# fightingnoble/rram-caffe-simulation

Measured on AMD Instinct MI355X. Metric: Monte Carlo fault-map inferences/sec, AlexNet b256, higher is better.
Workload: dtype f32 (bf16x6 products)

## Files before the change

rram-caffe-simulation_amd/csrc/x6.hip:

```cpp
#include <stdio.h>
#include <stdlib.h>
#include <string.h>

#include <algorithm>
#include <atomic>
#include <string>
#include <type_traits>

#include "gemm_common.hpp"
#include "split3.hpp"

namespace rram {
namespace {

#ifndef RRAM_X6_DROP
#define RRAM_X6_DROP 0
#endif
namespace x6 {
__device__ __forceinline__ floatx16 mfma6(const Parts& a, const Parts& b, floatx16 c) {
  if (RRAM_X6_DROP != 1) c = __builtin_amdgcn_mfma_f32_32x32x16_bf16(a.l, b.h, c, 0, 0, 0);
  if (RRAM_X6_DROP != 2) c = __builtin_amdgcn_mfma_f32_32x32x16_bf16(a.h, b.l, c, 0, 0, 0);
  if (RRAM_X6_DROP != 3) c = __builtin_amdgcn_mfma_f32_32x32x16_bf16(a.m, b.m, c, 0, 0, 0);
  if (RRAM_X6_DROP != 4) c = __builtin_amdgcn_mfma_f32_32x32x16_bf16(a.m, b.h, c, 0, 0, 0);
  if (RRAM_X6_DROP != 5) c = __builtin_amdgcn_mfma_f32_32x32x16_bf16(a.h, b.m, c, 0, 0, 0);
// ... 1059 lines not shown
  static_assert(NS * STB + 1024 <= 160 * 1024, "LDS");
  static_assert((NS - 2) * PPW <= 63, "vmcnt");
  __shared__ __attribute__((aligned(16))) char smem[NS * STB + 1024];
  const uint32_t lds0 = static_cast<uint32_t>(reinterpret_cast<uintptr_t>((__attribute__((address_space(3))) char*)smem));

  const int lane = threadIdx.x & 63;
  const int wave = __builtin_amdgcn_readfirstlane(threadIdx.x >> 6);
  const int lr = lane & 31, lh = lane >> 5;
  const int wr = wave % WR, wc = wave / WR;
  const int tid = xcd_tile_id(blockIdx.x, gridDim.x);
  const int tm = __builtin_amdgcn_readfirstlane(tid % P.tiles_m);
  const int tn = __builtin_amdgcn_readfirstlane(tid / P.tiles_m);
  const int m0 = tm * BMc, n0 = tn * BNc;
  const int HW = static_cast<int>(P.cv.howo.d), C = P.cv.C, KT = C >> 4;
  const int4v xrs = make_rsrc(x, xrange);
  const int4v wrs = make_rsrc(reinterpret_cast<const float*>(wpack), wrange);
  uint32_t aoff[PA], alds[PA];
#pragma unroll
  for (int i = 0; i < PA; ++i) {
    const int a = wave + 4 * i;
    const bool ok = a < NA;
    aoff[i] = ok ? static_cast<uint32_t>(((tm * RBL + a / 3) * KT) * 3072 + (a % 3) * 1024 + lane * 16) : 0x80000000u;
    alds[i] = ok ? static_cast<uint32_t>((a / 3 * 3 + a % 3) * 1024) : 0xFFFFFFFFu;
  }
  uint32_t boff[PB], blds[PB];
#pragma unroll
  for (int i = 0; i < PB; ++i) {
    const int q = wave + 4 * i;
    uint32_t off = 0x80000000u;
    if (q < NBP) {
      const int e = q * (PIECE_B / 4) + lane * 4;
      const int c = e / BNc, n = n0 + (e - c * BNc);
      if (n < P.N) {
        const uint32_t img = fdiv(static_cast<uint32_t>(n), P.cv.howo);
        const uint32_t sp = static_cast<uint32_t>(n) - img * static_cast<uint32_t>(HW);
        off = ((img * static_cast<uint32_t>(C) + static_cast<uint32_t>(c)) * static_cast<uint32_t>(HW) + sp) * 4u;
      }
    }
    boff[i] = off;
    blds[i] = q < NBP ? static_cast<uint32_t>(A_BYTES + q * PIECE_B) : 0xFFFFFFFFu;
  }
  const uint32_t kstep = static_cast<uint32_t>(HW) * 64u;
  auto issue = [&](int kt) {
    const bool ok = kt < KT;
    const uint32_t st = lds0 + static_cast<uint32_t>((kt % NS) * STB);
#pragma unroll
    for (int i = 0; i < PA; ++i) {
      const bool real = ok && alds[i] != 0xFFFFFFFFu;
      dma_b128(wrs, real ? aoff[i] + static_cast<uint32_t>(kt) * 3072u : 0x80000000u,
               real ? st + alds[i] : lds0 + static_cast<uint32_t>(NS * STB));
    }
#pragma unroll
    for (int i = 0; i < PB; ++i) {
      const bool real = ok && blds[i] != 0xFFFFFFFFu;
      const uint32_t vo = real && boff[i] != 0x80000000u ? boff[i] + static_cast<uint32_t>(kt) * kstep : 0x80000000u;
      const uint32_t dst = real ? st + blds[i] : lds0 + static_cast<uint32_t>(NS * STB);
      dma_b128(xrs, vo, dst);
    }
  };
  floatx16 acc[MI][NB];
#pragma unroll
  for (int i = 0; i < MI; ++i)
#pragma unroll
    for (int j = 0; j < NB; ++j)
#pragma unroll
      for (int r = 0; r < 16; ++r) acc[i][j][r] = 0.0f;

#pragma unroll
  for (int t = 0; t < NS - 1; ++t) issue(t);
  wait_vm<(NS - 2) * PPW>();
  __builtin_amdgcn_s_barrier();
  const int colw = 32 * NB * wc + lr;
  for (int kt = 0; kt < KT; ++kt) {
    issue(kt + NS - 1);
    const char* st = smem + (kt % NS) * STB;
    x6::Parts fa[MI];
#pragma unroll
    for (int i = 0; i < MI; ++i) {
      const char* f = st + (MI * wr + i) * 3072 + lane * 16;
      fa[i].h = *reinterpret_cast<const x6::bf16x8*>(f);
      fa[i].m = *reinterpret_cast<const x6::bf16x8*>(f + 1024);
      fa[i].l = *reinterpret_cast<const x6::bf16x8*>(f + 2048);
    }
    const float* bs = reinterpret_cast<const float*>(st + A_BYTES) + 8 * lh * BNc + colw;
#pragma unroll
    for (int j = 0; j < NB; ++j) {
      float v[8];
#pragma unroll
      for (int e = 0; e < 8; ++e) v[e] = bs[e * BNc + 32 * j];
      x6::Parts bp;
      x6::split8_safe(v, bp);
#pragma unroll
      for (int i = 0; i < MI; ++i) acc[i][j] = x6::mfma6(fa[i], bp, acc[i][j]);
    }
    wait_vm<(NS - 2) * PPW>();
    asm volatile("s_waitcnt lgkmcnt(0)" ::: "memory");
    __builtin_amdgcn_s_barrier();
    __builtin_amdgcn_sched_barrier(0);
  }
  Epi ep = P.e;
  conv_epilogue_nchw<MI, NB>(acc, P, ep, m0 + 32 * MI * wr, n0 + 32 * NB * wc, lr, lh);
  if (yoct != nullptr) octet_epilogue<MI, NB>(acc, P, ep, m0 + 32 * MI * wr, n0 + 32 * NB * wc, lr, lh, yoct, cout8);
}

__global__ void __launch_bounds__(256) k_conv_cb_pack_x6(const float* __restrict__ w, char* __restrict__ out, int M,
                                                         int Cg, int T, int rblocks, int units) {
  const int KT = Cg >> 4;
  for (int u = blockIdx.x * blockDim.x + threadIdx.x; u < units; u += gridDim.x * blockDim.x) {
    const int lane = u & 63;
    int r = u >> 6;
    const int s = r % T;
    r /= T;
    const int kt = r % KT;
    r /= KT;
    const int rb = r % rblocks;
    const int g = r / rblocks;
    const int m = rb * 32 + (lane & 31), c0 = kt * 16 + (lane >> 5) * 8;
    float v[8];
#pragma unroll
    for (int e = 0; e < 8; ++e)
      v[e] = m < M ? w[((int64_t)g * M + m) * Cg * T + (int64_t)(c0 + e) * T + s] : 0.0f;
    x6::Parts t;
    x6::split8_safe(v, t);
    char* f = out + (int64_t)(u >> 6) * 3072 + lane * 16;
    *reinterpret_cast<x6::bf16x8*>(f) = t.h;
    *reinterpret_cast<x6::bf16x8*>(f + 1024) = t.m;
    *reinterpret_cast<x6::bf16x8*>(f + 2048) = t.l;
  }
}


namespace c1x6 {
constexpr int BM = 96, BN = 256;
constexpr int KR = 11, KQ = 3, C = 3, NQ = C * KR * KQ, G = (NQ + 3) / 4;
constexpr int ROWS = 32;
constexpr int ROWE = 248;
constexpr int TERMB = ROWS * ROWE * 2;
constexpr int SLOTB = 3 * TERMB;
constexpr int QP = ROWE / 8;
constexpr int CHUNKS = ROWS * QP;
constexpr int CPT = (CHUNKS + 255) / 256;
static_assert(3 * SLOTB + BM * 4 <= 160 * 1024, "LDS");
constexpr int first_group(int c) { return (c * KR * KQ) / 4; }
constexpr int last_group(int c) { return (c * KR * KQ + KR * KQ - 1) / 4; }
constexpr int quad_off(int q) {
  return (q / (KR * KQ)) * SLOTB + (((q / KQ) % KR) * ROWE + 4 * (q % KQ)) * 2;
}
constexpr int half_delta(int q) { return q + 1 < NQ ? quad_off(q + 1) - quad_off(q) : 0; }
constexpr uint32_t hi_mask(int q) { return q >= NQ ? 0u : (q % KQ == KQ - 1 ? 0x0000FFFFu : 0xFFFFFFFFu); }
constexpr uint32_t lo_mask(int q) { return q >= NQ ? 0u : 0xFFFFFFFFu; }
}

template <int W>
__global__ void __launch_bounds__(256) __attribute__((amdgpu_waves_per_eu(1, 1)))
k_conv1_ring_x6(Params P, const uint16_t* __restrict__ wpack, int tiles_per_img, int tiles) {
  using namespace c1x6;
  constexpr int OW = (W - 11) / 4 + 1, MI = 3;
  static_assert(4 * (OW - 1) + 4 * KQ <= ROWE, "slot rows too short");
  __shared__ __attribute__((aligned(16))) char smem[3 * SLOTB];
  __shared__ float bias_lds[BM];
  if (threadIdx.x < BM)
    bias_lds[threadIdx.x] = (P.e.bias != nullptr && (int)threadIdx.x < P.M) ? P.e.bias[threadIdx.x] : 0.0f;
  const int lane = threadIdx.x & 63;
  const int wave = __builtin_amdgcn_readfirstlane(threadIdx.x >> 6);
  const int lr = lane & 31, lh = lane >> 5;
  const int HWo = P.cv.howo.d, H = P.cv.H;
  const int nwg = gridDim.x;
  const float* const xin = P.b.p;
  const int in_bytes = static_cast<int>(P.cv.in_bytes);

  float sv[2][8];
  struct TileRef {
    int img, f;
  };
  auto tile_ref = [&](int t) __attribute__((always_inline)) {
    TileRef r;
    const int img = t / tiles_per_img, tin = t - img * tiles_per_img;
    r.img = __builtin_amdgcn_readfirstlane(t < tiles ? img : -1);
    r.f = __builtin_amdgcn_readfirstlane((tin * BN) / OW);
    return r;
  };
  auto chunk_of = [&](int k) __attribute__((always_inline)) { return min((int)threadIdx.x + k * 256, CHUNKS - 1); };
  auto stage_load = [&](const TileRef& tr, int c, int k, float (&v)[8]) {
    const int q = chunk_of(k);
    const int ri = q / QP, qp = q - ri * QP;
    const bool ok = tr.img >= 0 && 4 * tr.f + ri < H;
    const int rowoff = (((tr.img * 3 + c) * H + 4 * tr.f + ri) * W + 8 * qp) * 4;
    const uint32_t voff = ok ? static_cast<uint32_t>(rowoff) : 0x80000000u;
    const __amdgpu_buffer_rsrc_t xrs =
        __builtin_amdgcn_make_buffer_rsrc(const_cast<float*>(xin), 0, in_bytes, 0x00020000);
#pragma unroll
    for (int e = 0; e < 8; ++e)
      v[e] = __builtin_bit_cast(float, __builtin_amdgcn_raw_buffer_load_b32(xrs, static_cast<int>(voff + 4 * e), 0, 0));
  };
  auto stage_store = [&](int c, int k, float (&v)[8]) {
    const int q = chunk_of(k);
    const int ri = q / QP, qp = q - ri * QP;
    const int nv = W - 8 * qp;
#pragma unroll
    for (int e = 0; e < 8; ++e) v[e] = e < nv ? v[e] : 0.0f;
    char* base = smem + c * SLOTB + (ri * ROWE + 8 * qp) * 2;
    x6::Parts t;
    x6::split8_safe(v, t);
    *reinterpret_cast<x6::bf16x8*>(base) = t.h;
    *reinterpret_cast<x6::bf16x8*>(base + TERMB) = t.m;
    *reinterpret_cast<x6::bf16x8*>(base + 2 * TERMB) = t.l;
  };
  auto fill_slot = [&](const TileRef& tr, int c) __attribute__((always_inline)) {
    for (int k = 0; k < CPT; ++k) {
      stage_load(tr, c, k, sv[0]);
      stage_store(c, k, sv[0]);
    }
  };

  const x6::bf16x8* ap = reinterpret_cast<const x6::bf16x8*>(wpack) + lane;
  auto launder_a = [&]() __attribute__((always_inline)) {
    int z = 0;
    asm volatile("" : "+s"(z));
    ap = reinterpret_cast<const x6::bf16x8*>(wpack) + lane + z;
  };
  auto load_a = [&](x6::bf16x8 (&f)[MI][3], int g) {
#pragma unroll
    for (int i = 0; i < MI; ++i)
#pragma unroll
      for (int tt = 0; tt < 3; ++tt) f[i][tt] = ap[((g * MI + i) * 3 + tt) * 64];
  };
  auto lds_barrier = [&]() __attribute__((always_inline)) {
    __builtin_amdgcn_s_waitcnt(0xC07F);
    __builtin_amdgcn_s_barrier();
  };

  int t = blockIdx.x;
  if (t < tiles) {
    const TileRef tr = tile_ref(t);
    fill_slot(tr, 0);
    fill_slot(tr, 1);
    fill_slot(tr, 2);
  }
  lds_barrier();
  floatx16 acc[2][MI][2];
  const __amdgpu_buffer_rsrc_t ors = __builtin_amdgcn_make_buffer_rsrc(P.e.C, 0, 0x7FFFFFFF, 0x00020000);
  const bool relu = P.e.relu != 0;
  const int mw = 4 * lh;
  uint32_t obase[2] = {0x80000000u, 0x80000000u};
  auto store_part = [&](const floatx16 (&pa)[MI][2], int s8) __attribute__((always_inline)) {
#pragma unroll
    for (int e = 0; e < 8; ++e) {
      const int v = 8 * s8 + e, i = (v >> 4) / 2, j = (v >> 4) & 1, r = v & 15;
      const int dr = i * 32 + (r & 3) + 8 * (r >> 2);
      const float o = pa[i][j][r] + bias_lds[mw + dr];
      __builtin_amdgcn_raw_buffer_store_b32(__builtin_bit_cast(uint32_t, relu ? fmaxf(o, 0.0f) : o), ors,
                                            static_cast<int>(obase[j]), dr * HWo * 4, 0);
    }
  };
  auto tile_body = [&](auto cc, int t) __attribute__((always_inline)) {
    constexpr int CUR = decltype(cc)::value;
    const TileRef cur = tile_ref(t), nxt = tile_ref(t + nwg);
    const int img = cur.img, sp0 = (t - img * tiles_per_img) * BN, f = cur.f;
    uint32_t lb[2];
#pragma unroll
    for (int j = 0; j < 2; ++j) {
      const int sp = min(sp0 + wave * 64 + j * 32 + lr, HWo - 1);
      const int oh = sp / OW, ow = sp - oh * OW;
      lb[j] = static_cast<uint32_t>((4 * (oh - f) * ROWE + 4 * ow) * 2);
    }
    typedef uint32_t u32x2 __attribute__((ext_vector_type(2)));
    typedef uint32_t u32x4 __attribute__((ext_vector_type(4)));
    auto pick = [&](uint32_t h0, uint32_t h1) __attribute__((always_inline)) { return lh ? h1 : h0; };
    auto mask_q = [&](u32x2 v, int q0) __attribute__((always_inline)) {
      if (lo_mask(q0) != 0xFFFFFFFFu || lo_mask(q0 + 1) != 0xFFFFFFFFu) v[0] &= pick(lo_mask(q0), lo_mask(q0 + 1));
      if (hi_mask(q0) != 0xFFFFFFFFu || hi_mask(q0 + 1) != 0xFFFFFFFFu) v[1] &= pick(hi_mask(q0), hi_mask(q0 + 1));
      return v;
    };
    auto read_part = [&](x6::Parts (&F)[2], int g, int part) __attribute__((always_inline)) {
      const int j = part / 3, tt = part % 3;
      const int qa = 4 * g, qb = 4 * g + 2;
      const char* ba = smem + lb[j] + (lh ? half_delta(qa) : 0) + tt * TERMB;
      const char* bb = smem + lb[j] + (lh ? half_delta(qb) : 0) + tt * TERMB;
      const u32x2 lo = mask_q(*reinterpret_cast<const u32x2*>(ba + quad_off(qa)), qa);
      const u32x2 hi = mask_q(*reinterpret_cast<const u32x2*>(bb + quad_off(qb)), qb);
      const x6::bf16x8 v = __builtin_bit_cast(x6::bf16x8, u32x4{lo[0], lo[1], hi[0], hi[1]});
      if (tt == 0) F[j].h = v;
      else if (tt == 1) F[j].m = v;
      else F[j].l = v;
    };
    floatx16 (&ac)[MI][2] = acc[CUR];
    const floatx16 (&ap_)[MI][2] = acc[1 - CUR];
#pragma unroll
    for (int i = 0; i < MI; ++i)
#pragma unroll
      for (int j = 0; j < 2; ++j)
#pragma unroll
        for (int r = 0; r < 16; ++r) ac[i][j][r] = 0.0f;
    x6::bf16x8 fg[3][MI][3];
    launder_a();
    load_a(fg[0], 0);
    load_a(fg[1], 1);
    x6::Parts F[2][2];
#pragma unroll
    for (int part = 0; part < 6; ++part) read_part(F[0], 0, part);
    static_for<0, G>([&](auto gc) {
      constexpr int g = decltype(gc)::value;
      x6::Parts (&fc)[2] = F[g & 1];
      x6::Parts (&fn)[2] = F[(g + 1) & 1];
      if (g + 2 < G) load_a(fg[(g + 2) % 3], g + 2);
      auto refill1 = [&](const TileRef& tr, int c, int st) __attribute__((always_inline)) {
        if (st > 0 && st - 1 < CPT) stage_store(c, st - 1, sv[(st - 1) & 1]);
        if (st < CPT) stage_load(tr, c, st, sv[st & 1]);
      };
      auto refill = [&]() __attribute__((always_inline)) {
        if (g >= 1 && g <= 1 + CPT) refill1(cur, 2, g - 1);
        constexpr int d0 = g - last_group(0) - 1, d1 = g - last_group(1) - 1;
        if (d0 >= 0 && d0 <= CPT) refill1(nxt, 0, d0);
        if (d1 >= 0 && d1 <= CPT) refill1(nxt, 1, d1);
      };
#pragma unroll
      for (int q = 0; q < 2 * MI; ++q) {
        const int i = q >> 1, j = q & 1;
        const auto& fa = fg[g % 3][i];
        ac[i][j] = x6::mfma6(x6::Parts{fa[0], fa[1], fa[2]}, fc[j], ac[i][j]);
        if (g + 1 < G) read_part(fn, g + 1, q);
        if (q == 1) refill();
        if (g < 12 && q == 3) store_part(ap_, g);
#pragma unroll
        for (int k = 0; k < 6; ++k) {
          __builtin_amdgcn_sched_group_barrier(0x008, 1, 0);
          __builtin_amdgcn_sched_group_barrier(0x100, 1, 0);
          __builtin_amdgcn_sched_group_barrier(0x002, 4, 0);
          __builtin_amdgcn_sched_group_barrier(0x200, 1, 0);
          __builtin_amdgcn_sched_group_barrier(0x020, 3, 0);
          __builtin_amdgcn_sched_group_barrier(0x040, 1, 0);
        }
        __builtin_amdgcn_sched_barrier(0);
      }
      if (g == last_group(0) || g == last_group(1) || g == G - 1) lds_barrier();
    });
#pragma unroll
    for (int j = 0; j < 2; ++j) {
      const int sp = sp0 + wave * 64 + j * 32 + lr;
      obase[j] = sp < HWo ? static_cast<uint32_t>(((int64_t)img * P.e.cimg + sp + (int64_t)mw * HWo) * 4)
                          : 0x80000000u;
    }
  };
  for (; t < tiles; t += 2 * nwg) {
    tile_body(std::integral_constant<int, 0>{}, t);
    if (t + nwg >= tiles) {
#pragma unroll
      for (int s8 = 0; s8 < 12; ++s8) store_part(acc[0], s8);
      return;
    }
    tile_body(std::integral_constant<int, 1>{}, t + nwg);
  }
  if (t - nwg < tiles && t != (int)blockIdx.x) {
#pragma unroll
    for (int s8 = 0; s8 < 12; ++s8) store_part(acc[1], s8);
  }
}

__global__ void __launch_bounds__(256) k_conv1_pack_x6(const float* __restrict__ w, char* __restrict__ out, int M,
                                                       int units) {
  using namespace c1x6;
  for (int u = blockIdx.x * blockDim.x + threadIdx.x; u < units; u += gridDim.x * blockDim.x) {
    const int lane = u & 63, i = (u >> 6) % 3, g = (u >> 6) / 3;
    const int row = 32 * i + (lane & 31), h = lane >> 5;
    float v[8];
#pragma unroll
    for (int j = 0; j < 8; ++j) {
      const int q = 4 * g + 2 * (j >> 2) + h;
      const int c = q / (KR * KQ), kh = (q / KQ) % KR, kw = 4 * (q % KQ) + (j & 3);
      v[j] = (row < M && q < NQ && kw < 11) ? w[((row * 3 + c) * 11 + kh) * 11 + kw] : 0.0f;
    }
    x6::Parts t;
    x6::split8_safe(v, t);
    char* f = out + (int64_t)(u >> 6) * 3072 + lane * 16;
    *reinterpret_cast<x6::bf16x8*>(f) = t.h;
    *reinterpret_cast<x6::bf16x8*>(f + 1024) = t.m;
    *reinterpret_cast<x6::bf16x8*>(f + 2048) = t.l;
  }
}

namespace c7x6 {
constexpr int C = 3, KS = 7, S = 2, KC = 8;
constexpr int R = C * KS;
constexpr int G = (R + 1) / 2;
constexpr int BM = 64, MI = 2;
constexpr int ROWE = 232;
constexpr int QR = ROWE / 4;
static_assert((ROWE * 2) % 8 == 0, "8-byte staging stores");
template <int NBW>
struct Tile {
  static constexpr int BN = 128 * NBW;
  static constexpr int OR = NBW == 2 ? 4 : 3;
  static constexpr int SR = S * (OR - 1) + KS;
  static constexpr int TERMB = SR * ROWE * 2;
  static constexpr int CHB = 3 * TERMB;
  static constexpr int NCH = C * SR * QR;
  static constexpr int CPT = (NCH + 255) / 256;
  static constexpr int WGS = NBW == 2 ? 2 : 3;
  static_assert(WGS * (C * CHB + BM * 4) <= 160 * 1024, "LDS");
  static constexpr int row_off(int rr) { return rr < R ? (rr / KS) * CHB + (rr % KS) * ROWE * 2 : 0; }
};
}

template <int NBW>
__global__ void __launch_bounds__(256) __attribute__((amdgpu_waves_per_eu(NBW == 2 ? 2 : 3, NBW == 2 ? 2 : 3)))
k_conv_s2_x6(Params P, const x6::bf16x8* __restrict__ wpack, int tiles_per_img, int tiles) {
  using namespace c7x6;
  using T = Tile<NBW>;
  constexpr int BN = T::BN, SR = T::SR, TERMB = T::TERMB, CHB = T::CHB, NCH = T::NCH, CPT = T::CPT;
  __shared__ __attribute__((aligned(16))) char smem[C * CHB];
  __shared__ float bias_lds[BM];
  const int lane = threadIdx.x & 63;
  const int wave = __builtin_amdgcn_readfirstlane(threadIdx.x >> 6);
  const int lr = lane & 31, lh = lane >> 5;
  const int t = __builtin_amdgcn_readfirstlane(xcd_tile_id(blockIdx.x, gridDim.x));
  if (t >= tiles) return;
  const int img = t / tiles_per_img, sp0 = (t - img * tiles_per_img) * BN;
  const int HWo = P.cv.howo.d, OW = P.cv.Wo, H = P.cv.H, W = P.cv.W;
  const int f = sp0 / OW;
  if (threadIdx.x < BM)
    bias_lds[threadIdx.x] = (P.e.bias != nullptr && (int)threadIdx.x < P.M) ? P.e.bias[threadIdx.x] : 0.0f;

  {
    const __amdgpu_buffer_rsrc_t xrs =
        __builtin_amdgcn_make_buffer_rsrc(const_cast<float*>(P.b.p), 0, static_cast<int>(P.cv.in_bytes), 0x00020000);
    const int row0 = S * f - P.cv.ph;
    float v[CPT][4];
#pragma unroll
    for (int k = 0; k < CPT; ++k) {
      const int q = min((int)threadIdx.x + 256 * k, NCH - 1);
      const int c = q / (SR * QR), rem = q - c * (SR * QR), ri = rem / QR, e4 = rem - ri * QR;
      const int row = row0 + ri, col0 = 4 * e4 - P.cv.pw;
      const bool rok = static_cast<unsigned>(row) < static_cast<unsigned>(H);
      const int base = ((img * C + c) * H + row) * W + col0;
#pragma unroll
      for (int e = 0; e < 4; ++e) {
        const bool ok = rok && static_cast<unsigned>(col0 + e) < static_cast<unsigned>(W);
        v[k][e] = __builtin_bit_cast(
            float, __builtin_amdgcn_raw_buffer_load_b32(xrs, ok ? 4 * (base + e) : static_cast<int>(0x80000000u), 0, 0));
      }
    }
#pragma unroll
    for (int k = 0; k < CPT; ++k) {
      const int q = min((int)threadIdx.x + 256 * k, NCH - 1);
      const int c = q / (SR * QR), rem = q - c * (SR * QR), ri = rem / QR, e4 = rem - ri * QR;
      typedef uint32_t u32x2 __attribute__((ext_vector_type(2)));
      u32x2 hw, mw, lw;
#pragma unroll
      for (int p = 0; p < 2; ++p) {
        const x6::float2v xv = {v[k][2 * p], v[k][2 * p + 1]};
        x6::bf16x2 h;
        const x6::float2v r1 = x6::bf16_high_safe(xv, h);
        const x6::bf16x2 m = __builtin_convertvector(x6::clamp_bf16(r1), x6::bf16x2);
        const x6::float2v r2 = r1 - __builtin_convertvector(m, x6::float2v);
        const x6::bf16x2 l = __builtin_convertvector(r2, x6::bf16x2);
        hw[p] = __builtin_bit_cast(uint32_t, h);
        mw[p] = __builtin_bit_cast(uint32_t, m);
        lw[p] = __builtin_bit_cast(uint32_t, l);
      }
      char* dst = smem + c * CHB + (ri * ROWE + 4 * e4) * 2;
      *reinterpret_cast<u32x2*>(dst) = hw;
      *reinterpret_cast<u32x2*>(dst + TERMB) = mw;
      *reinterpret_cast<u32x2*>(dst + 2 * TERMB) = lw;
    }
  }
  __syncthreads();

  uint32_t lb[NBW];
#pragma unroll
  for (int j = 0; j < NBW; ++j) {
    const int sp = min(sp0 + wave * 32 * NBW + j * 32 + lr, HWo - 1);
    const int oh = sp / OW, ow = sp - oh * OW;
    lb[j] = static_cast<uint32_t>((S * (oh - f) * ROWE + S * ow) * 2);
  }
  const x6::bf16x8* ap = wpack + lane;
  auto load_a = [&](x6::bf16x8 (&fr)[MI][3], int g) __attribute__((always_inline)) {
#pragma unroll
    for (int i = 0; i < MI; ++i)
#pragma unroll
      for (int tt = 0; tt < 3; ++tt) fr[i][tt] = ap[((g * MI + i) * 3 + tt) * 64];
  };
  typedef uint32_t u32x4 __attribute__((ext_vector_type(4)));
  auto read_b = [&](u32x4 (&Bq)[NBW][3], int g) __attribute__((always_inline)) {
    const uint32_t ho = lh ? static_cast<uint32_t>(T::row_off(2 * g + 1)) : static_cast<uint32_t>(T::row_off(2 * g));
#pragma unroll
    for (int j = 0; j < NBW; ++j)
#pragma unroll
      for (int tt = 0; tt < 3; ++tt) {
        const uint32_t* p = reinterpret_cast<const uint32_t*>(smem + lb[j] + ho + tt * TERMB);
        Bq[j][tt] = u32x4{p[0], p[1], p[2], p[3]};
      }
  };
  auto parts_b = [&](const u32x4 (&Bq)[NBW][3], int j, int g) __attribute__((always_inline)) {
    const uint32_t m3 = (2 * g + 1 < R || lh == 0) ? 0x0000FFFFu : 0u;
    const uint32_t m02 = (2 * g + 1 < R || lh == 0) ? 0xFFFFFFFFu : 0u;
    x6::bf16x8 t[3];
#pragma unroll
    for (int tt = 0; tt < 3; ++tt) {
      u32x4 d = Bq[j][tt];
      asm volatile("" : "+v"(d));
      if (2 * g + 1 >= R) {
        d[0] &= m02;
        d[1] &= m02;
        d[2] &= m02;
      }
      d[3] &= m3;
      t[tt] = __builtin_bit_cast(x6::bf16x8, d);
    }
    return x6::Parts{t[0], t[1], t[2]};
// ... 314 lines not shown
    for (int j = 0; j < 8; ++j) v[j] = 0.0f;
    const float* p0 = ws + (int64_t)m * N + n0;
    int z = 0;
    for (; z + 8 <= split; z += 8) {
      float4 q[8][2];
#pragma unroll
      for (int zz = 0; zz < 8; ++zz) {
        q[zz][0] = *reinterpret_cast<const float4*>(p0 + (int64_t)(z + zz) * total);
        q[zz][1] = *reinterpret_cast<const float4*>(p0 + (int64_t)(z + zz) * total + 4);
      }
#pragma unroll
      for (int zz = 0; zz < 8; ++zz) {
        v[0] += q[zz][0].x; v[1] += q[zz][0].y; v[2] += q[zz][0].z; v[3] += q[zz][0].w;
        v[4] += q[zz][1].x; v[5] += q[zz][1].y; v[6] += q[zz][1].z; v[7] += q[zz][1].w;
      }
    }
    for (; z < split; ++z) {
      const float4 a = *reinterpret_cast<const float4*>(p0 + (int64_t)z * total);
      const float4 b = *reinterpret_cast<const float4*>(p0 + (int64_t)z * total + 4);
      v[0] += a.x; v[1] += a.y; v[2] += a.z; v[3] += a.w;
      v[4] += b.x; v[5] += b.y; v[6] += b.z; v[7] += b.w;
    }
#pragma unroll
    for (int j = 0; j < 8; ++j) {
      const int n = n0 + j;
      float o = ep.alpha * v[j];
      if (ep.bias_mode == RRAM_BIAS_ROW) o += ep.bias[m];
      else if (ep.bias_mode == RRAM_BIAS_COL) o += ep.bias[n];
      if (ep.relu) o = fmaxf(o, 0.0f);
      v[j] = o;
    }
    float* dst = ep.C + (int64_t)m * ep.ldc + n0;
    *reinterpret_cast<float4*>(dst) = make_float4(v[0], v[1], v[2], v[3]);
    *reinterpret_cast<float4*>(dst + 4) = make_float4(v[4], v[5], v[6], v[7]);
    const int kt = n0 >> 5, kk = n0 & 31, h = kk >> 4, g = (kk >> 3) & 1;
    const int tm = m / BMc, row = m - tm * BMc;
    char* rowp = pack + (((int64_t)tm * ktiles + kt) * BMc + row) * gx6::RLB;
    x6::store_terms8(v, rowp + (g * 2 + h) * 48);
    if (g == 1 && h == 1) *reinterpret_cast<uint4*>(rowp + 192) = make_uint4(0, 0, 0, 0);
  }
}

}

float* pack_buffer(size_t floats, hipStream_t s);

constexpr bool fits_i32(int64_t count, int elem_bytes = 1) { return count * elem_bytes < (1ll << 31); }

int patch_rows(int N, int HW, int OW, int OH, int KH, int BN, int maxseg) {
  int rmax = 0;
  for (int n0 = 0; n0 < N; n0 += BN) {
    const int pl = std::min(n0 + BN, N) - 1;
    const int i0 = n0 / HW, i1 = pl / HW;
    if (i1 - i0 + 1 > maxseg) return -1;
    int r = 0;
    for (int i = i0; i <= i1; ++i) {
      const int f = i == i0 ? (n0 - i0 * HW) / OW : 0;
      const int l = i == i1 ? (pl - i1 * HW) / OW : OH - 1;
      r += l - f + KH;
    }
    rmax = std::max(rmax, r);
  }
  return rmax;
}

Params conv_params(const rram_conv_desc* d, const WPack& wk, float* y, const float* bias, int relu) {
  const int Cg = d->channels / d->group, HW = d->out_h * d->out_w;
  Params P{};
  P.M = d->num_output / d->group;
  P.N = d->num * HW;
  P.K = Cg * d->kernel_h * d->kernel_w;
  P.split = 1;
  P.cv.C = Cg;
  P.cv.howo = make_fastdiv(HW);
  P.e = make_epi(y, HW, 1.0f, 0.0f, bias, RRAM_BIAS_ROW, relu);
  P.e.cimg = wk.y_img > 0 ? wk.y_img : (int64_t)d->num_output * HW;
  P.e.hw = make_fastdiv(HW);
  return P;
}
void conv_window(const rram_conv_desc* d, ConvGeom& cv) {
  cv.H = d->height;
  cv.W = d->width;
  cv.KH = d->kernel_h;
  cv.KW = d->kernel_w;
  cv.ph = d->pad_h;
  cv.pw = d->pad_w;
  cv.sh = d->stride_h;
  cv.sw = d->stride_w;
  cv.dh = d->dilation_h;
  cv.dw = d->dilation_w;
  cv.Ho = d->out_h;
  cv.Wo = d->out_w;
  cv.wo_div = make_fastdiv(d->out_w);
}
void conv_input_view(const rram_conv_desc* d, const float* x, Params& P) {
  P.b = make_view(x, 0, P.N, P.K);
  P.cv.chw = (int64_t)d->channels * d->height * d->width;
  P.cv.in_bytes = static_cast<int>((int64_t)d->num * P.cv.chw * 4);
}

template <class PackW, class PackLead>
int conv_weight_pack(const WPack& wk, int64_t wbytes, hipStream_t s, const char* what, PackW pack_w, char** wbuf,
                     int64_t lead, PackLead pack_lead) {
  if (wk.query) {
    *wk.query = static_cast<size_t>(wbytes);
    return 1;
  }
  const int64_t scratch = lead + (wk.p ? 0 : wbytes);
  char* buf = scratch > 0 ? reinterpret_cast<char*>(pack_buffer(static_cast<size_t>((scratch + 3) / 4), s)) : nullptr;
  RRAM_REQUIRE(scratch == 0 || buf != nullptr, "conv: packed-operand buffer allocation failed");
  *wbuf = wk.p ? static_cast<char*>(wk.p) : buf + lead;
  int rc = pack_lead(buf);
  if (rc == 0 && !wk.valid) {
    pack_w(*wbuf);
    rc = launch_status(what);
  }
  return rc;
}
template <class PackW>
int conv_weight_pack(const WPack& wk, int64_t wbytes, hipStream_t s, const char* what, PackW pack_w, char** wbuf) {
  return conv_weight_pack(wk, wbytes, s, what, pack_w, wbuf, 0, [](char*) { return 0; });
}


bool conv1_ring_ok(const rram_conv_desc* d) {
  return d->group == 1 && d->channels == 3 && d->kernel_h == 11 && d->kernel_w == 11 && d->stride_h == 4 &&
         d->stride_w == 4 && d->pad_h == 0 && d->pad_w == 0 && d->dilation_h == 1 && d->dilation_w == 1 &&
         d->width == 227 && d->height >= 11 && d->num_output == c1x6::BM && d->num > 0 &&
         fits_i32((int64_t)d->num * 3 * d->height * d->width, 4) &&
         fits_i32((int64_t)d->num * d->num_output * d->out_h * d->out_w, 4);
}

int conv_wide_x6_fwd(const rram_conv_desc* d, const float* x, const float* w, const float* bias, float* y, int relu,
                     hipStream_t s, const WPack& wk) {
  const int HW = d->out_h * d->out_w;
  Params P = conv_params(d, wk, y, bias, relu);
  conv_window(d, P.cv);
  conv_input_view(d, x, P);
  if (!fits_i32((int64_t)d->num * P.e.cimg, 4)) return 0;
  const int units = c1x6::G * 3 * 64;
  char* wp = nullptr;
  if (const int rc = conv_weight_pack(
          wk, (int64_t)units * 48, s, "conv1 weight pack x6",
          [&](char* p) {
            hipLaunchKernelGGL(k_conv1_pack_x6, dim3(stream_blocks(units)), dim3(256), 0, s, w, p, d->num_output, units);
          },
          &wp))
    return rc;
  const int tpi = (HW + c1x6::BN - 1) / c1x6::BN;
  const int tiles = d->num * tpi;
  int cus = 256;
  (void)hipDeviceGetAttribute(&cus, hipDeviceAttributeMultiprocessorCount, 0);
  const unsigned nwg = static_cast<unsigned>(std::min(tiles, cus));
  hipLaunchKernelGGL((k_conv1_ring_x6<227>), dim3(nwg), dim3(256), 0, s, P, reinterpret_cast<const uint16_t*>(wp),
                     tpi, tiles);
  const int rc = launch_status("conv1 ring x6");
  return rc ? rc : 1;
}

constexpr int kS2Nbw = 2;
bool conv_s2_ok(const rram_conv_desc* d) {
  namespace k = c7x6;
  using T = k::Tile<kS2Nbw>;
  return d->group == 1 && d->channels == k::C && d->kernel_h == k::KS && d->kernel_w == k::KS &&
         d->stride_h == k::S && d->stride_w == k::S && d->dilation_h == 1 && d->dilation_w == 1 && d->pad_h >= 0 &&
         d->pad_h <= 3 && d->pad_w >= 0 && d->pad_w <= 3 && d->num_output >= 1 && d->num_output <= k::BM &&
         d->num > 0 && d->out_w >= 85 && d->out_h >= 1 && k::S * (d->out_w - 1) + k::KC <= k::ROWE &&
         (d->out_w + T::BN - 2) / d->out_w <= T::OR - 1 &&
         fits_i32((int64_t)d->num * k::C * d->height * d->width, 4) &&
         fits_i32((int64_t)d->num * d->num_output * d->out_h * d->out_w, 4);
}

int conv_s2_x6_fwd(const rram_conv_desc* d, const float* x, const float* w, const float* bias, float* y, int relu,
                   hipStream_t s, const WPack& wk) {
  const int HW = d->out_h * d->out_w;
  Params P = conv_params(d, wk, y, bias, relu);
  conv_window(d, P.cv);
  conv_input_view(d, x, P);
  if (!fits_i32((int64_t)d->num * P.e.cimg, 4)) return 0;
  const int units = c7x6::G * c7x6::MI * 64;
  char* wp = nullptr;
  if (const int rc = conv_weight_pack(
          wk, (int64_t)units * 48, s, "conv s2 weight pack x6",
          [&](char* p) {
            hipLaunchKernelGGL(k_conv_s2_pack_x6, dim3(stream_blocks(units)), dim3(256), 0, s, w, p, d->num_output,
                               units);
          },
          &wp))
    return rc;
  const int tpi = (HW + c7x6::Tile<kS2Nbw>::BN - 1) / c7x6::Tile<kS2Nbw>::BN;
  const int64_t tiles = (int64_t)d->num * tpi;
  RRAM_REQUIRE(fits_i32(tiles), "conv: grid too large");
  hipLaunchKernelGGL(k_conv_s2_x6<kS2Nbw>, dim3(static_cast<unsigned>(tiles)), dim3(256), 0, s, P,
                     reinterpret_cast<const x6::bf16x8*>(wp), tpi, static_cast<int>(tiles));
  const int rc = launch_status("conv s2 x6");
  return rc ? rc : 1;
}

std::atomic<int>& f32_engine() {
  static std::atomic<int> eng{[] {
    const char* e = getenv("RRAM_X6");
    return (e && atoi(e) == 0) ? static_cast<int>(RRAM_ENGINE_F32) : static_cast<int>(RRAM_ENGINE_BF16X6);
  }()};
  return eng;
}

struct ConvPlan {
  int CPH, MI, mt, PW, CS, PD;
};
#define RRAM_PATCH_LIST(X) \
  X(5, 1, 4) X(5, 1, 8) X(5, 1, 12) X(3, 4, 8) X(3, 4, 12) X(3, 4, 16) X(3, 2, 4) X(3, 2, 8) X(3, 2, 16)
struct PatchForm {
  int KH, CPH, PD;
};
constexpr PatchForm kPatchForms[] = {
#define RRAM_X(kh, cph, pd) {kh, cph, pd},
    RRAM_PATCH_LIST(RRAM_X)
#undef RRAM_X
};
int patch_pd(int KH, int CPH, int need) {
  int pd = 0;
  for (const PatchForm& f : kPatchForms)
    if (f.KH == KH && f.CPH == CPH && f.PD >= need && (pd == 0 || f.PD < pd)) pd = f.PD;
  return pd;
}
bool patch_built(int KH, int CPH, int PD) { return PD > 0 && patch_pd(KH, CPH, PD) == PD; }
bool conv_x6_plan(const rram_conv_desc* d, ConvPlan& pl) {
  const int KH = d->kernel_h, KW = d->kernel_w;
  if (d->stride_h != 1 || d->stride_w != 1 || d->dilation_h != 1 || d->dilation_w != 1) return false;
  if (!((KH == 3 && KW == 3) || (KH == 5 && KW == 5))) return false;
  const int G = d->group, Cg = d->channels / G, M = d->num_output / G;
  const int HW = d->out_h * d->out_w, OW = d->out_w, OH = d->out_h;
  pl.CPH = KH == 5 ? 1 : (Cg % 8 == 0 ? 4 : 2);
  if (HW < 128 || Cg == 0 || Cg % (2 * pl.CPH) != 0) return false;
  if (!fits_i32((int64_t)d->num * d->channels * d->height * d->width, 4)) return false;
  if (!fits_i32((int64_t)d->num * d->num_output * HW, 4)) return false;
  const int t128 = (M + 127) / 128 * 128, t96 = (M + 95) / 96 * 96;
  pl.MI = (t96 - M) < (t128 - M) ? 3 : 4;
  pl.mt = pl.MI == 3 ? t96 : t128;
  if ((pl.mt - M) * 8 > pl.mt) return false;
  const int rmax = patch_rows(d->num * HW, HW, OW, OH, KH, x6::BN, 3);
  if (rmax < 0) return false;
  pl.PW = d->width + 2 * d->pad_w;
  pl.CS = rmax * pl.PW;
  while ((pl.CPH * pl.CS) % 64 != 32) ++pl.CS;
  pl.PD = patch_pd(KH, pl.CPH, (2 * pl.CPH * pl.CS + 255) / 256);
  if (pl.PD == 0) return false;
  const int64_t total = (int64_t)G * (pl.mt / (32 * pl.MI)) * (Cg / (2 * pl.CPH)) * 32 * pl.MI *
                        (((KH * KW * pl.CPH + 7) / 8 * 96 + 16) / 2);
  return fits_i32(total, 2);
}

template <int KH, int CPH, int MI, int PD>
int launch_patch_x6(Params P, const uint16_t* wpack, int PW, int CS, int gz, hipStream_t s) {
  P.tiles_m = (P.M + 32 * MI - 1) / (32 * MI);
  P.tiles_n = (P.N + x6::BN - 1) / x6::BN;
  P.tiles_z = gz;
  const int64_t nwg = (int64_t)P.tiles_m * P.tiles_n * gz;
  RRAM_REQUIRE(fits_i32(nwg), "conv: grid too large");
  hipLaunchKernelGGL((k_conv_patch_x6<KH, KH, CPH, MI, PD>), dim3(static_cast<unsigned>(nwg)), dim3(256), 0, s, P, wpack,
                     PW, CS);
  return launch_status("conv patch x6");
}

int conv_patch_x6_fwd(const rram_conv_desc* d, const ConvPlan& pl, const float* x, const float* w, const float* bias,
                      float* y, int relu, hipStream_t s, const WPack& wk) {
  const int KH = d->kernel_h, T = KH * d->kernel_w;
  const int G = d->group, Cg = d->channels / G, M = d->num_output / G;
  const int CPH = pl.CPH, MI = pl.MI, PW = pl.PW, CS = pl.CS, PD = pl.PD;
  Params P = conv_params(d, wk, y, bias, relu);
  conv_window(d, P.cv);
  conv_input_view(d, x, P);
  P.grp_b = (int64_t)Cg * d->height * d->width;
  P.grp_c = (int64_t)M * d->out_h * d->out_w;
  P.grp_bias = M;
  const int S = CPH * T, G8 = (S + 7) / 8, RLH = (G8 * 96 + 16) / 2;
  const int BMc = 32 * MI, tiles_m = pl.mt / BMc, ktiles = Cg / (2 * CPH);
  const int64_t total = (int64_t)G * tiles_m * ktiles * BMc * RLH;
  char* wbuf = nullptr;
  if (const int rc = conv_weight_pack(
          wk, total * 2, s, "conv weight pack x6",
          [&](char* p) {
            const int units = G * tiles_m * ktiles * BMc * G8 * 2;
            hipLaunchKernelGGL(k_conv_patch_pack_x6, dim3(stream_blocks(units)), dim3(256), 0, s, w, p, G, M, Cg, T,
                               CPH, G8, 2 * RLH, BMc, tiles_m, ktiles, units);
          },
          &wbuf))
    return rc;
  const uint16_t* wp = reinterpret_cast<const uint16_t*>(wbuf);
  int rc = 0;
#define RRAM_P(KH_, CPH_, PD_)                                                                           \
  if (KH == KH_ && CPH == CPH_ && PD == PD_)                                                             \
    rc = MI == 3 ? launch_patch_x6<KH_, CPH_, 3, PD_>(P, wp, PW, CS, G, s)                               \
                 : launch_patch_x6<KH_, CPH_, 4, PD_>(P, wp, PW, CS, G, s);                              \
  else
  RRAM_PATCH_LIST(RRAM_P)
  RRAM_REQUIRE(false, "conv: the plan names a patch kernel that is not built");
#undef RRAM_P
  return rc ? rc : 1;
}

int pack_octets(const float* x, void* oct, int num, int C, int HWi, hipStream_t s) {
  RRAM_REQUIRE(C % 8 == 0 && fits_i32((int64_t)num * C * HWi, 6), "pack_octets: C %% 8 != 0 or too large");
  const int units = num * (C / 8) * HWi;
  if (units == 0) return RRAM_OK;
  hipLaunchKernelGGL(k_pack_octets_x6, dim3(stream_blocks(units)), dim3(256), 0, s, x, static_cast<char*>(oct), C / 8,
                     HWi, units);
// ... 670 lines not shown
```

Measured before the change: 136,400.

## Warp-specialize conv1 ring kernel with producer waves filling LDS slots

Doubles the conv1 workgroup to 512 threads. Four extra producer waves load input rows, split them into bf16 terms and write the LDS ring slots, while the four consumer waves only run MFMAs. Tiles are now assigned as contiguous ranges per workgroup instead of strided. A rotating five-entry register ring of weight fragments replaces the per-group triple buffer, and the single accumulator set's stores are folded into the first group of the next tile. The aim is to take global loads and the split work off the MFMA waves' critical path and lower register pressure. The cost is two waves per EU, more barriers per tile (the two roles must stay in lockstep on barrier count), and a scheduling change.

```diff
diff --git a/rram-caffe-simulation_amd/csrc/x6.hip b/rram-caffe-simulation_amd/csrc/x6.hip
--- a/rram-caffe-simulation_amd/csrc/x6.hip
+++ b/rram-caffe-simulation_amd/csrc/x6.hip
@@ -1235,110 +1235,128 @@
 }
 
 template <int W>
-__global__ void __launch_bounds__(256) __attribute__((amdgpu_waves_per_eu(1, 1)))
+__global__ void __launch_bounds__(512) __attribute__((amdgpu_waves_per_eu(2, 2)))
 k_conv1_ring_x6(Params P, const uint16_t* __restrict__ wpack, int tiles_per_img, int tiles) {
   using namespace c1x6;
   constexpr int OW = (W - 11) / 4 + 1, MI = 3;
+  constexpr int NF = G * MI, FR = 5;
   static_assert(4 * (OW - 1) + 4 * KQ <= ROWE, "slot rows too short");
+  static_assert(NF % FR == 0, "the fragment ring must close over a tile");
   __shared__ __attribute__((aligned(16))) char smem[3 * SLOTB];
   __shared__ float bias_lds[BM];
   if (threadIdx.x < BM)
     bias_lds[threadIdx.x] = (P.e.bias != nullptr && (int)threadIdx.x < P.M) ? P.e.bias[threadIdx.x] : 0.0f;
   const int lane = threadIdx.x & 63;
   const int wave = __builtin_amdgcn_readfirstlane(threadIdx.x >> 6);
-  const int lr = lane & 31, lh = lane >> 5;
   const int HWo = P.cv.howo.d, H = P.cv.H;
-  const int nwg = gridDim.x;
-  const float* const xin = P.b.p;
-  const int in_bytes = static_cast<int>(P.cv.in_bytes);
-
-  float sv[2][8];
+  const int nwg = gridDim.x, wg = blockIdx.x;
+  const int per = tiles / nwg, rem = tiles - per * nwg;
+  const int t0 = wg * per + min(wg, rem), t1 = t0 + per + (wg < rem ? 1 : 0);
   struct TileRef {
     int img, f;
   };
   auto tile_ref = [&](int t) __attribute__((always_inline)) {
     TileRef r;
     const int img = t / tiles_per_img, tin = t - img * tiles_per_img;
-    r.img = __builtin_amdgcn_readfirstlane(t < tiles ? img : -1);
+    r.img = __builtin_amdgcn_readfirstlane(t < t1 ? img : -1);
     r.f = __builtin_amdgcn_readfirstlane((tin * BN) / OW);
     return r;
   };
-  auto chunk_of = [&](int k) __attribute__((always_inline)) { return min((int)threadIdx.x + k * 256, CHUNKS - 1); };
-  auto stage_load = [&](const TileRef& tr, int c, int k, float (&v)[8]) {
-    const int q = chunk_of(k);
-    const int ri = q / QP, qp = q - ri * QP;
-    const bool ok = tr.img >= 0 && 4 * tr.f + ri < H;
-    const int rowoff = (((tr.img * 3 + c) * H + 4 * tr.f + ri) * W + 8 * qp) * 4;
-    const uint32_t voff = ok ? static_cast<uint32_t>(rowoff) : 0x80000000u;
-    const __amdgpu_buffer_rsrc_t xrs =
-        __builtin_amdgcn_make_buffer_rsrc(const_cast<float*>(xin), 0, in_bytes, 0x00020000);
-#pragma unroll
-    for (int e = 0; e < 8; ++e)
-      v[e] = __builtin_bit_cast(float, __builtin_amdgcn_raw_buffer_load_b32(xrs, static_cast<int>(voff + 4 * e), 0, 0));
-  };
-  auto stage_store = [&](int c, int k, float (&v)[8]) {
-    const int q = chunk_of(k);
-    const int ri = q / QP, qp = q - ri * QP;
-    const int nv = W - 8 * qp;
-#pragma unroll
-    for (int e = 0; e < 8; ++e) v[e] = e < nv ? v[e] : 0.0f;
-    char* base = smem + c * SLOTB + (ri * ROWE + 8 * qp) * 2;
-    x6::Parts t;
-    x6::split8_safe(v, t);
-    *reinterpret_cast<x6::bf16x8*>(base) = t.h;
-    *reinterpret_cast<x6::bf16x8*>(base + TERMB) = t.m;
-    *reinterpret_cast<x6::bf16x8*>(base + 2 * TERMB) = t.l;
-  };
-  auto fill_slot = [&](const TileRef& tr, int c) __attribute__((always_inline)) {
-    for (int k = 0; k < CPT; ++k) {
-      stage_load(tr, c, k, sv[0]);
-      stage_store(c, k, sv[0]);
-    }
-  };
-
+  auto lds_barrier = [&]() __attribute__((always_inline)) {
+    __builtin_amdgcn_s_waitcnt(0xC07F);
+    __builtin_amdgcn_s_barrier();
+  };
+
+  if (wave >= 4) {
+    const float* const xin = P.b.p;
+    const int in_bytes = static_cast<int>(P.cv.in_bytes);
+    const int ptid = static_cast<int>(threadIdx.x) - 256;
+    auto fill_slot = [&](const TileRef& tr, int c) __attribute__((always_inline)) {
+      const __amdgpu_buffer_rsrc_t xrs =
+          __builtin_amdgcn_make_buffer_rsrc(const_cast<float*>(xin), 0, in_bytes, 0x00020000);
+      float v[CPT][8];
+#pragma unroll
+      for (int k = 0; k < CPT; ++k) {
+        const int q = min(ptid + k * 256, CHUNKS - 1);
+        const int ri = q / QP, qp = q - ri * QP;
+        const bool ok = 4 * tr.f + ri < H;
+        const int rowoff = (((tr.img * 3 + c) * H + 4 * tr.f + ri) * W + 8 * qp) * 4;
+        const uint32_t voff = ok ? static_cast<uint32_t>(rowoff) : 0x80000000u;
+#pragma unroll
+        for (int e = 0; e < 8; ++e)
+          v[k][e] =
+              __builtin_bit_cast(float, __builtin_amdgcn_raw_buffer_load_b32(xrs, static_cast<int>(voff + 4 * e), 0, 0));
+      }
+#pragma unroll
+      for (int k = 0; k < CPT; ++k) {
+        const int q = min(ptid + k * 256, CHUNKS - 1);
+        const int ri = q / QP, qp = q - ri * QP;
+        const int nv = W - 8 * qp;
+#pragma unroll
+        for (int e = 0; e < 8; ++e) v[k][e] = e < nv ? v[k][e] : 0.0f;
+        char* base = smem + c * SLOTB + (ri * ROWE + 8 * qp) * 2;
+        x6::Parts t;
+        x6::split8_safe(v[k], t);
+        *reinterpret_cast<x6::bf16x8*>(base) = t.h;
+        *reinterpret_cast<x6::bf16x8*>(base + TERMB) = t.m;
+        *reinterpret_cast<x6::bf16x8*>(base + 2 * TERMB) = t.l;
+      }
+    };
+    TileRef cur = tile_ref(t0);
+    fill_slot(cur, 0);
+    fill_slot(cur, 1);
+    lds_barrier();
+    for (int t = t0; t < t1; ++t) {
+      const TileRef nxt = tile_ref(t + 1);
+      fill_slot(cur, 2);
+      lds_barrier();
+      if (nxt.img >= 0) fill_slot(nxt, 0);
+      lds_barrier();
+      if (nxt.img >= 0) fill_slot(nxt, 1);
+      lds_barrier();
+      cur = nxt;
+    }
+    return;
+  }
+
+  const int lr = lane & 31, lh = lane >> 5;
   const x6::bf16x8* ap = reinterpret_cast<const x6::bf16x8*>(wpack) + lane;
   auto launder_a = [&]() __attribute__((always_inline)) {
     int z = 0;
     asm volatile("" : "+s"(z));
     ap = reinterpret_cast<const x6::bf16x8*>(wpack) + lane + z;
   };
-  auto load_a = [&](x6::bf16x8 (&f)[MI][3], int g) {
-#pragma unroll
-    for (int i = 0; i < MI; ++i)
-#pragma unroll
-      for (int tt = 0; tt < 3; ++tt) f[i][tt] = ap[((g * MI + i) * 3 + tt) * 64];
-  };
-  auto lds_barrier = [&]() __attribute__((always_inline)) {
-    __builtin_amdgcn_s_waitcnt(0xC07F);
-    __builtin_amdgcn_s_barrier();
-  };
-
-  int t = blockIdx.x;
-  if (t < tiles) {
-    const TileRef tr = tile_ref(t);
-    fill_slot(tr, 0);
-    fill_slot(tr, 1);
-    fill_slot(tr, 2);
-  }
-  lds_barrier();
-  floatx16 acc[2][MI][2];
+  x6::bf16x8 fs[FR][3];
+  auto load_frag = [&](int s) __attribute__((always_inline)) {
+#pragma unroll
+    for (int tt = 0; tt < 3; ++tt) fs[s % FR][tt] = ap[(s * 3 + tt) * 64];
+  };
+  floatx16 acc[MI][2];
+#pragma unroll
+  for (int i = 0; i < MI; ++i)
+#pragma unroll
+    for (int j = 0; j < 2; ++j)
+#pragma unroll
+      for (int r = 0; r < 16; ++r) acc[i][j][r] = 0.0f;
   const __amdgpu_buffer_rsrc_t ors = __builtin_amdgcn_make_buffer_rsrc(P.e.C, 0, 0x7FFFFFFF, 0x00020000);
   const bool relu = P.e.relu != 0;
   const int mw = 4 * lh;
   uint32_t obase[2] = {0x80000000u, 0x80000000u};
-  auto store_part = [&](const floatx16 (&pa)[MI][2], int s8) __attribute__((always_inline)) {
-#pragma unroll
-    for (int e = 0; e < 8; ++e) {
-      const int v = 8 * s8 + e, i = (v >> 4) / 2, j = (v >> 4) & 1, r = v & 15;
+  auto store_block = [&](int i, int j) __attribute__((always_inline)) {
+#pragma unroll
+    for (int r = 0; r < 16; ++r) {
       const int dr = i * 32 + (r & 3) + 8 * (r >> 2);
-      const float o = pa[i][j][r] + bias_lds[mw + dr];
+      const float o = acc[i][j][r] + bias_lds[mw + dr];
       __builtin_amdgcn_raw_buffer_store_b32(__builtin_bit_cast(uint32_t, relu ? fmaxf(o, 0.0f) : o), ors,
                                             static_cast<int>(obase[j]), dr * HWo * 4, 0);
     }
   };
-  auto tile_body = [&](auto cc, int t) __attribute__((always_inline)) {
-    constexpr int CUR = decltype(cc)::value;
-    const TileRef cur = tile_ref(t), nxt = tile_ref(t + nwg);
+  launder_a();
+#pragma unroll
+  for (int s = 0; s < FR - 1; ++s) load_frag(s);
+  lds_barrier();
+  for (int t = t0; t < t1; ++t) {
+    const TileRef cur = tile_ref(t);
     const int img = cur.img, sp0 = (t - img * tiles_per_img) * BN, f = cur.f;
     uint32_t lb[2];
 #pragma unroll
@@ -1367,18 +1385,7 @@
       else if (tt == 1) F[j].m = v;
       else F[j].l = v;
     };
-    floatx16 (&ac)[MI][2] = acc[CUR];
-    const floatx16 (&ap_)[MI][2] = acc[1 - CUR];
-#pragma unroll
-    for (int i = 0; i < MI; ++i)
-#pragma unroll
-      for (int j = 0; j < 2; ++j)
-#pragma unroll
-        for (int r = 0; r < 16; ++r) ac[i][j][r] = 0.0f;
-    x6::bf16x8 fg[3][MI][3];
     launder_a();
-    load_a(fg[0], 0);
-    load_a(fg[1], 1);
     x6::Parts F[2][2];
 #pragma unroll
     for (int part = 0; part < 6; ++part) read_part(F[0], 0, part);
@@ -1386,33 +1393,28 @@
       constexpr int g = decltype(gc)::value;
       x6::Parts (&fc)[2] = F[g & 1];
       x6::Parts (&fn)[2] = F[(g + 1) & 1];
-      if (g + 2 < G) load_a(fg[(g + 2) % 3], g + 2);
-      auto refill1 = [&](const TileRef& tr, int c, int st) __attribute__((always_inline)) {
-        if (st > 0 && st - 1 < CPT) stage_store(c, st - 1, sv[(st - 1) & 1]);
-        if (st < CPT) stage_load(tr, c, st, sv[st & 1]);
-      };
-      auto refill = [&]() __attribute__((always_inline)) {
-        if (g >= 1 && g <= 1 + CPT) refill1(cur, 2, g - 1);
-        constexpr int d0 = g - last_group(0) - 1, d1 = g - last_group(1) - 1;
-        if (d0 >= 0 && d0 <= CPT) refill1(nxt, 0, d0);
-        if (d1 >= 0 && d1 <= CPT) refill1(nxt, 1, d1);
-      };
 #pragma unroll
       for (int q = 0; q < 2 * MI; ++q) {
-        const int i = q >> 1, j = q & 1;
-        const auto& fa = fg[g % 3][i];
-        ac[i][j] = x6::mfma6(x6::Parts{fa[0], fa[1], fa[2]}, fc[j], ac[i][j]);
+        const int i = q >> 1, j = q & 1, s = g * MI + i;
+        if (j == 0) load_frag((s + FR - 1) % NF);
+        const auto& fa = fs[s % FR];
+        if (g == 0) {
+          store_block(i, j);
+          floatx16 z;
+#pragma unroll
+          for (int r = 0; r < 16; ++r) z[r] = 0.0f;
+          acc[i][j] = x6::mfma6(x6::Parts{fa[0], fa[1], fa[2]}, fc[j], z);
+        } else {
+          acc[i][j] = x6::mfma6(x6::Parts{fa[0], fa[1], fa[2]}, fc[j], acc[i][j]);
+        }
         if (g + 1 < G) read_part(fn, g + 1, q);
-        if (q == 1) refill();
-        if (g < 12 && q == 3) store_part(ap_, g);
 #pragma unroll
         for (int k = 0; k < 6; ++k) {
           __builtin_amdgcn_sched_group_barrier(0x008, 1, 0);
           __builtin_amdgcn_sched_group_barrier(0x100, 1, 0);
-          __builtin_amdgcn_sched_group_barrier(0x002, 4, 0);
-          __builtin_amdgcn_sched_group_barrier(0x200, 1, 0);
+          __builtin_amdgcn_sched_group_barrier(0x002, g == 0 ? 10 : 4, 0);
           __builtin_amdgcn_sched_group_barrier(0x020, 3, 0);
-          __builtin_amdgcn_sched_group_barrier(0x040, 1, 0);
+          if (g == 0) __builtin_amdgcn_sched_group_barrier(0x040, 3, 0);
         }
         __builtin_amdgcn_sched_barrier(0);
       }
@@ -1424,20 +1426,9 @@
       obase[j] = sp < HWo ? static_cast<uint32_t>(((int64_t)img * P.e.cimg + sp + (int64_t)mw * HWo) * 4)
                           : 0x80000000u;
     }
-  };
-  for (; t < tiles; t += 2 * nwg) {
-    tile_body(std::integral_constant<int, 0>{}, t);
-    if (t + nwg >= tiles) {
-#pragma unroll
-      for (int s8 = 0; s8 < 12; ++s8) store_part(acc[0], s8);
-      return;
-    }
-    tile_body(std::integral_constant<int, 1>{}, t + nwg);
-  }
-  if (t - nwg < tiles && t != (int)blockIdx.x) {
-#pragma unroll
-    for (int s8 = 0; s8 < 12; ++s8) store_part(acc[1], s8);
-  }
+  }
+#pragma unroll
+  for (int q = 0; q < 2 * MI; ++q) store_block(q >> 1, q & 1);
 }
 
 __global__ void __launch_bounds__(256) k_conv1_pack_x6(const float* __restrict__ w, char* __restrict__ out, int M,
@@ -2058,7 +2049,7 @@
   int cus = 256;
   (void)hipDeviceGetAttribute(&cus, hipDeviceAttributeMultiprocessorCount, 0);
   const unsigned nwg = static_cast<unsigned>(std::min(tiles, cus));
-  hipLaunchKernelGGL((k_conv1_ring_x6<227>), dim3(nwg), dim3(256), 0, s, P, reinterpret_cast<const uint16_t*>(wp),
+  hipLaunchKernelGGL((k_conv1_ring_x6<227>), dim3(nwg), dim3(512), 0, s, P, reinterpret_cast<const uint16_t*>(wp),
                      tpi, tiles);
   const int rc = launch_status("conv1 ring x6");
   return rc ? rc : 1;
```

Result: no change. 137,700 (median of 6 runs) (+0.9%).
